# kokutoupan/burn_raymarching

Hardware: AMD Instinct MI355X
Metric: Mrays/s fwd+bwd, 512x512 / 256 spheres / 32 steps, at 1/2/4/8 MI355X (higher is better)
Workload: dtype f32

## Files before the change

burn_raymarching_amd/csrc/rm_kernels.hip:

```cpp
#include <hip/hip_runtime.h>
#include <hip/hip_ext.h>

#include <algorithm>
#include <cstdarg>
#include <cmath>
#include <cstdio>
#include <cstdlib>
#include <cstring>
#include <string>
#include <type_traits>
#include <utility>
#include <vector>

#include "../../include/raymarch.h"
#include "rm_device.h"

namespace rm {

constexpr int kOrderClasses = 16;
constexpr int kOrderClsStride = 32;
constexpr int kOrderCntStride = kOrderClasses * kOrderClsStride > 64 ? kOrderClasses * kOrderClsStride : 64;
static_assert(kOrderCntStride >= kOrderClasses * kOrderClsStride && kOrderCntStride % 32 == 0, "128-byte lines per set");
constexpr int kRedArrStride = 32;

enum Mode { kFwd = 0, kBwd = 1, kTrain = 2, kRender = 3 };

constexpr int kMaxBlocksPerLaunch = 131072 * (256 / kBlock);
constexpr int kInlineCams = 16;
constexpr int kSplitMinSpheres = 256;
constexpr int kSplitMinSpheresWide = 512;
constexpr long long kSplitMaxRaysWide = 1048576;
constexpr int kSplitMinWaves = 3;
constexpr int kSplitWaves = 4;
static_assert(kSplitWaves == 2 || kSplitWaves == 4, "split blocks have 2 or 4 waves");
constexpr int kSplitRays = 32;
static_assert(kSplitRays == 64 || kSplitRays == 32 || kSplitRays == 16, "split blocks hold 64, 32 or 16 rays");
constexpr int kSplitCB = kSplitRays / 16;
constexpr long long kSplitMaxRays = 262144;
constexpr int kReduceSegs = 128;

struct KArgs {
  const float* org;
  const float* dir;
  long long ray_begin;
  long long n_rays;
  int width, height, num_views;
  int tiling;
  int cull;
  float cull_min_d;
  float lse_slack;
  unsigned long long* stats;
  float gone_d;
  int early_exit;
  int split;
  int mfma;
  int shift_max;
  const int* esc_flags;
  const int* block_order;
  int order_views, order_tiles;
  const int* olist_r;
  const int* ocnt_r;
  int* olist_w;
  int* ocnt_w;
  int* ocnt_z;
  const int* oturn;
  CamBasis cams[kInlineCams];
  const CamBasis* cams_dev;
  const float* centers;
  const float* colors;
  const _Float16* colors_h;
  const float* radius;
  const float* light_dir;
  const float* ambient;
  int M, Mpad;
  const float4* rec_buf;
  float* origin;
  int steps;
  float k, eps, csharp, msharp;
  float* out;
  float* t_out;
  const float* t_in;
  const float* gout;
  const float* targets;
  float progress, inv_count;
  const rm_step_scalars* sdev;
  float light_fixed[3];
  float* dbg;
  float* partials;
  long long rec;
  int cont_cap, cont_resume;
  float* cont_state;
  const int* cont_list;
  const int* cont_count;
  int* cont_list_w;
  int* cont_count_w;
  long long cont_rays;
  int ray_cont;
  const int* ray_list;
  const int* ray_count;
  int* ray_list_w;
  int* ray_count_w;
#ifdef RM_BLOCK_TRACE
  unsigned long long* btrace;
#endif
};
#ifdef RM_BLOCK_TRACE
constexpr int kTraceWords = 12;
__device__ __forceinline__ void trace_word(const KArgs& a, int w, unsigned long long v) {
  if (a.btrace != nullptr && (threadIdx.x & 63) == 0)
    a.btrace[kTraceWords * ((unsigned long long)blockIdx.x * kWaves + (threadIdx.x >> 6)) + w] = v;
}
#define RM_TRACE(w, v) trace_word(a, (w), (v))
#else
#define RM_TRACE(w, v) ((void)0)
#endif

typedef float f4v __attribute__((ext_vector_type(4)));
typedef float f2v __attribute__((ext_vector_type(2)));
typedef const __attribute__((address_space(4))) f4v* cf4_ptr;
typedef const __attribute__((address_space(4))) f2v* cf2_ptr;
typedef const __attribute__((address_space(4))) float* cf1_ptr;

constexpr int kRecHeader = 8;

__host__ __device__ inline size_t tiles_offset(int npairs, int nprep) {
  return ((size_t)npairs * (7 * 16 + 8) + (size_t)(nprep + 1) * kRecHeader * sizeof(float) + 15) & ~(size_t)15;
}
constexpr int kEscTab = 64;
constexpr int kStatsWords = 6;
__host__ __device__ inline size_t esc_offset(int npairs, int nprep) {
  const size_t nrb = (size_t)npairs / 8;
  return tiles_offset(npairs, nprep) + nrb * 64 * 16 + nrb * 32 * sizeof(float);
}
__host__ __device__ inline size_t origin_offset(int npairs, int nprep) {
  return esc_offset(npairs, nprep) + kEscTab * sizeof(float);
}
// ... 81 lines not shown
      v[k] = fminf(v[k], c);
      v[3 + k] = fmaxf(v[3 + k], c);
    }
#pragma unroll
  for (int off = 32; off > 0; off >>= 1)
#pragma unroll
    for (int k = 0; k < 3; ++k) {
      v[k] = fminf(v[k], __shfl_xor(v[k], off));
      v[3 + k] = fmaxf(v[3 + k], __shfl_xor(v[3 + k], off));
    }
  if (lane == 0)
#pragma unroll
    for (int k = 0; k < 6; ++k) scratch[8 * wave + k] = v[k];
  __syncthreads();
#pragma unroll
  for (int k = 0; k < 3; ++k) {
    float lo = scratch[k], hi = scratch[3 + k];
    for (int w = 1; w < nw; ++w) {
      lo = fminf(lo, scratch[8 * w + k]);
      hi = fmaxf(hi, scratch[8 * w + 3 + k]);
    }
    c0[k] = 0.5f * (lo + hi);
  }
  float r = 0.0f;
  for (int j = tid; j < a.M; j += nt) {
    const float dx = a.centers[3 * j] - c0[0], dy = a.centers[3 * j + 1] - c0[1], dz = a.centers[3 * j + 2] - c0[2];
    r = fmaxf(r, fsqrt(dx * dx + dy * dy + dz * dz) + a.radius[j]);
  }
#pragma unroll
  for (int off = 32; off > 0; off >>= 1) r = fmaxf(r, __shfl_xor(r, off));
  __syncthreads();
  if (lane == 0) scratch[8 * wave] = r;
  __syncthreads();
  R = scratch[0];
  for (int w = 1; w < nw; ++w) R = fmaxf(R, scratch[8 * w]);
  R = R * (1.0f + 1e-5f) + 1e-6f;
  __syncthreads();
}

typedef short bf16x8 __attribute__((ext_vector_type(8)));
typedef float f32x4 __attribute__((ext_vector_type(4)));

__device__ __forceinline__ void split3(float x, unsigned& h1, unsigned& h2, unsigned& h3) {
  const unsigned a = __float_as_uint(x) & 0xFFFF0000u;
  const float r1 = x - __uint_as_float(a);
  const unsigned b = __float_as_uint(r1) & 0xFFFF0000u;
  const float r2 = r1 - __uint_as_float(b);
  const unsigned c = __float_as_uint(r2) & 0xFFFF0000u;
  h1 = a >> 16;
  h2 = b >> 16;
  h3 = c >> 16;
}
__device__ __forceinline__ unsigned pack2(unsigned lo16, unsigned hi16) { return lo16 | (hi16 << 16); }
constexpr unsigned kBf16One = 0x3F80u;

__device__ __forceinline__ uint4 mfma_a_slice(const KArgs& a, int j, int g) {
  const float kappa = a.k * kLog2e, k2 = kappa * kappa;
  float cx, cy, cz;
  if (j < a.M) {
    cx = a.centers[3 * j];
    cy = a.centers[3 * j + 1];
    cz = a.centers[3 * j + 2];
  } else {
    cx = kPadCenter;
    cy = cz = 0.0f;
  }
  unsigned x[3], y[3], z[3], C[3];
  split3(-2.0f * k2 * cx, x[0], x[1], x[2]);
  split3(-2.0f * k2 * cy, y[0], y[1], y[2]);
  split3(-2.0f * k2 * cz, z[0], z[1], z[2]);
  split3(k2 * (cx * cx + cy * cy + cz * cz), C[0], C[1], C[2]);
  if (g < 2)
    return make_uint4(pack2(x[g], x[g]), pack2(x[g], y[g]), pack2(y[g], y[g]), pack2(z[g], z[g]));
  if (g == 2) return make_uint4(pack2(x[2], x[2]), pack2(0u, y[2]), pack2(y[2], 0u), pack2(z[2], z[2]));
  return make_uint4(pack2(z[0], z[1]), pack2(kBf16One, kBf16One), pack2(kBf16One, C[0]), pack2(C[1], C[2]));
}
__device__ __forceinline__ uint4 mfma_a_frag(const KArgs& a, int e) {
  const int l = e & 63;
  return mfma_a_slice(a, 16 * (e >> 6) + (l & 15), l >> 4);
}
__device__ __forceinline__ int mfma_w_sphere(int e) { return 16 * (e >> 5) + (e & 15); }
__device__ __forceinline__ bool mfma_w_fixed(int e) { return (e & 16) != 0; }

__device__ void write_bound(const KArgs& a, float* hdr, float* esc) {
  __shared__ float scratch[8 * 16];
  float c[3], R;
  scene_bound(a, scratch, threadIdx.x, c, R);
  if (threadIdx.x == 0) {
    hdr[4] = c[0];
    hdr[5] = c[1];
    hdr[6] = c[2];
    hdr[7] = R;
  }
  if (threadIdx.x < kEscTab) {
    float tv = INFINITY;
    if (a.gone_d > 0.0f) {
      const float rp = (R + a.lse_slack + 1e-3f) * (1.0f + 1e-6f);
      const float inv_shrink = 1.0000101f;
      float T = (a.gone_d + rp) * (1.0f + 1e-6f);
      const float two_c2 = 2.0f * inv_shrink * inv_shrink * (1.0f + 1e-6f), nrp2 = -rp * rp,
                  half_up = 0.5f * (1.0f + 1e-5f);
      const int nmax = min((int)threadIdx.x, a.steps);
      for (int n = 1; n <= nmax; ++n) T = fmaf(rp + fsqrt(fmaf(two_c2 * T, T, nrp2)), half_up, 1e-6f);
      tv = T * (1.0f + 1e-6f);
    }
    esc[threadIdx.x] = tv;
  }
}

constexpr int kPrepStageMax = 512;

template <bool PAR>
__device__ void write_origins(const KArgs& a, const float4& S00, const float4& S10, float rmax, float spread,
                              const uint4* At, const float* Wt, float* orig, unsigned char* xch, int v);

__global__ __launch_bounds__(256) void rm_prep_kernel(const KArgs a0, float4* __restrict__ rec) {
  __shared__ float stage[7 * kPrepStageMax];
  const int nt = (int)blockDim.x;
  KArgs a = a0;
  if (gridDim.x == 1 && a0.M <= kPrepStageMax) {
    const int M = a0.M;
    for (int e = threadIdx.x; e < 3 * M; e += nt) {
      stage[e] = a0.centers[e];
      stage[3 * M + e] = a0.colors_h != nullptr ? (float)a0.colors_h[e] : a0.colors[e];
    }
    for (int e = threadIdx.x; e < M; e += nt) stage[6 * M + e] = a0.radius[e];
    __syncthreads();
    a.centers = stage;
    a.colors = stage + 3 * M;
    a.colors_h = nullptr;
    a.radius = stage + 6 * M;
  }
  const int np = a.Mpad / 2;
  float4* P0 = rec;
  float4* P1 = P0 + np;
  float4* P2 = P1 + np;
  float4* P3 = P2 + np;
  float4* S0 = P3 + np;
  float4* S1 = S0 + np;
  float4* W = S1 + np;
  float2* P4 = reinterpret_cast<float2*>(W + np);
  float* hdr = reinterpret_cast<float*>(P4 + np);
  const float kappa = a.k * kLog2e, k2 = kappa * kappa;
  const float kr_first = kappa * a.radius[0];
  const float c0x = a.centers[0], c0y = a.centers[1], c0z = a.centers[2];
  float rmin = INFINITY, rmax = 0.0f, spread = 0.0f;
  const int ip = blockIdx.x * nt + threadIdx.x;
  if (ip < np) {
    float gx[2], gy[2], gz[2], cc[2], kr[2], rr[2], cr[2], cg[2], cb[2], w[2], wf[2];
#pragma unroll
    for (int h = 0; h < 2; ++h) {
      const int j = 2 * ip + h;
      if (j < a.M) {
        const float cx = a.centers[3 * j], cy = a.centers[3 * j + 1], cz = a.centers[3 * j + 2];
        const float r = a.radius[j];
        gx[h] = -2.0f * cx;
        gy[h] = -2.0f * cy;
        gz[h] = -2.0f * cz;
        cc[h] = cx * cx + cy * cy + cz * cz;
        kr[h] = kappa * r;
        rr[h] = r;
        if (a.colors_h != nullptr) {
          cr[h] = (float)a.colors_h[3 * j];
          cg[h] = (float)a.colors_h[3 * j + 1];
          cb[h] = (float)a.colors_h[3 * j + 2];
        } else {
          cr[h] = a.colors[3 * j];
          cg[h] = a.colors[3 * j + 1];
          cb[h] = a.colors[3 * j + 2];
        }
        w[h] = fexp2(kr[h]);
// ... 755 lines not shown
```

burn_raymarching_amd/csrc/rm_launch.h:

```cpp
#pragma once

namespace {

using namespace rm;

int pad_spheres(int M) { return (M + kSphereAlign - 1) / kSphereAlign * kSphereAlign; }
constexpr int kRedArrivals = (RM_MAX_SPHERES * 8 + 8 + 255) / 256 * kRedArrStride;

long long max_blocks_per_launch() {
  const char* e = std::getenv("RM_MAX_BLOCKS_PER_LAUNCH");
  const long long v = e ? std::atoll(e) : 0;
  return (v >= 1 && v <= kMaxBlocksPerLaunch) ? v : kMaxBlocksPerLaunch;
}

long long rec_floats(int Mpad) { return (long long)Mpad * 8 + 8; }

int split_cont_steps(int steps) {
  if (const char* e = std::getenv("RM_SPLIT_CONT_STEPS")) return std::max(0, std::atoi(e));
  return steps >= 64 ? std::max(32, 3 * steps / 8) : 0;
}
int split_cont2_steps(int steps) {
  if (const char* e = std::getenv("RM_SPLIT_CONT2_STEPS")) return std::max(0, std::atoi(e));
  return steps >= 128 ? 3 * steps / 4 : 0;
}
// ... 433 lines not shown
}

int small_lpr(const Call& c, long long n) {
  if (c.mode != kTrain || env_is("RM_SMALL_LPR", '1')) return 1;
  return env_is("RM_SMALL_LPR", '2') || n <= 32768 ? 2 : 1;
}

int run_small(rm_context* ctx, const Call& c, KArgs& a, long long n) {
  const bool has_bwd = c.has_bwd();
  const int lpr = small_lpr(c, n), rpb = kBlock / lpr;
  int rc;
  if (has_bwd && (rc = ctx->ws.ensure(ctx, ws_need(n, a.M, rpb), "workspace")) != RM_OK) return rc;
  if ((rc = ctx->arrivals.ensure(ctx, 64, "arrival counter", true)) != RM_OK) return rc;
  long long done = 0;
  bool first = true;
  while (done < n) {
    const long long nb = std::min<long long>((n - done + rpb - 1) / rpb, max_blocks_per_launch());
    const long long nr = std::min<long long>(n - done, nb * rpb);
    a.ray_begin = done;
    a.n_rays = nr;
    a.partials = ctx->ws.as<float>();
#ifdef RM_BLOCK_TRACE
    if ((rc = bind_block_trace(ctx, a, (nb + (c.fused && c.fused->adam ? 1 : 0)) * kWaves)) != RM_OK) return rc;
    RM_HIP(ctx, hipMemsetAsync(a.btrace, 0, sizeof(unsigned long long) * kTraceWords * kWaves * (size_t)(nb + 1), ctx->stream));
#endif
    SmallArgs sa;
    std::memset(&sa, 0, sizeof sa);
    if (c.fused) sa = *c.fused;
    if (has_bwd) sa.fin = final_args(c, first);
    sa.arrivals = ctx->arrivals.as<unsigned>();
    sa.final_in_kernel = has_bwd && nb <= kSmallFinalMaxBlocks ? 1 : 0;
    if (c.fused && (!sa.final_in_kernel || nr != n))
      return fail(ctx, RM_ERR_INVALID_ARG, "fused iteration needs one launch of <= %d blocks", kSmallFinalMaxBlocks);
    const bool extra = c.fused && sa.adam;
    if (ctx->stats_dev) {
      ctx->stats_blocks += nb;
      ctx->stats_waves += nb * kWaves;
    }
    if (extra) {
      if ((rc = ctx->opt_pre.ensure(ctx, sizeof(float) * (4 * kOptPreStride + 2), "optimizer hand-off")) != RM_OK)
        return rc;
      sa.opt_pre = ctx->opt_pre.as<float>();
      ctx->opt_prepared = false;
    }
    hipEvent_t ev0, ev1;
    if ((rc = next_events(ctx, ev0, ev1)) != RM_OK) return rc;
    const dim3 grid((unsigned)(nb + (extra ? 1 : 0)));
    if (c.fused && lpr == 2) launch_small_m<kTrain, true, 2>(a.M, grid, ctx->stream, a, sa, ev0, ev1);
    else if (c.fused) launch_small_m<kTrain, true>(a.M, grid, ctx->stream, a, sa, ev0, ev1);
    else if (c.mode == kFwd) launch_small_m<kFwd>(a.M, grid, ctx->stream, a, sa, ev0, ev1);
    else if (c.mode == kBwd) launch_small_m<kBwd>(a.M, grid, ctx->stream, a, sa, ev0, ev1);
    else if (lpr == 2) launch_small_m<kTrain, false, 2>(a.M, grid, ctx->stream, a, sa, ev0, ev1);
    else launch_small_m<kTrain>(a.M, grid, ctx->stream, a, sa, ev0, ev1);
    RM_HIP(ctx, hipGetLastError());
    if (has_bwd && !sa.final_in_kernel && (rc = reduce_and_finalize(ctx, c, a, nb, first)) != RM_OK) return rc;
    done += nr;
    first = false;
  }
  return RM_OK;
}


template <int MODE>
void launch_escape(bool cam, dim3 grid, hipStream_t st, const KArgs& a, int* flags) {
  if (cam)
    hipLaunchKernelGGL((rm_escape_kernel<MODE, true>), grid, dim3(kBlock), 0, st, a, flags);
  else
    hipLaunchKernelGGL((rm_escape_kernel<MODE, false>), grid, dim3(kBlock), 0, st, a, flags);
}

template <int MODE>
bool launch_ray(bool cam, bool split, dim3 grid, size_t lds, hipStream_t st, const KArgs& a, hipEvent_t ev0,
                hipEvent_t ev1) {
  const dim3 blk(split ? 64 * kSplitWaves : kBlock);
  const uint32_t sh = (uint32_t)lds;
  if (split) {
    if constexpr (MODE == kRender) {
      return false;
    } else {
      if (cam) hipExtLaunchKernelGGL((rm_ray_kernel<MODE, true, true>), grid, blk, sh, st, ev0, ev1, 0u, a);
      else hipExtLaunchKernelGGL((rm_ray_kernel<MODE, false, true>), grid, blk, sh, st, ev0, ev1, 0u, a);
    }
  } else {
    if (cam) hipExtLaunchKernelGGL((rm_ray_kernel<MODE, true, false>), grid, blk, sh, st, ev0, ev1, 0u, a);
    else hipExtLaunchKernelGGL((rm_ray_kernel<MODE, false, false>), grid, blk, sh, st, ev0, ev1, 0u, a);
  }
  return true;
}

int check_call(rm_context* ctx, const Call& c, long long n) {
  if ((c.mode == kFwd || c.mode == kRender) && n > 0 && !c.out && !c.t_out && !c.dbg) return fail(ctx, RM_ERR_INVALID_ARG, "no output requested");
  if (c.mode == kBwd && n > 0 && !c.gout) return fail(ctx, RM_ERR_INVALID_ARG, "grad_out is NULL");
  if (c.mode == kTrain && n > 0 && !c.targets) return fail(ctx, RM_ERR_INVALID_ARG, "targets is NULL");
  if (c.has_bwd() && !c.grads) return fail(ctx, RM_ERR_INVALID_ARG, "grads is NULL");
  return RM_OK;
}

bool march_policy(const Call& c, long long n, KArgs& a) {
  const int M = a.M;
  const bool mask_vanishes = c.mode == kRender || a.msharp > 0.0f;
  bool split = false;
  if (c.mode != kRender && (c.march->flags & RM_MARCH_SKIP_ESCAPED) == 0) {
    const char* e = std::getenv("RM_SPLIT");
    if ((c.march->flags & RM_MARCH_SPLIT) != 0 || (e && e[0] == '1')) split = true;
    else if ((c.march->flags & RM_MARCH_NO_SPLIT) == 0 && !(e && e[0] == '0'))
      split = (M >= kSplitMinSpheres && n <= kSplitMaxRays) || (M >= kSplitMinSpheresWide && n <= kSplitMaxRaysWide);
  }
  a.split = split ? 1 : 0;
  a.cull = ((c.march->flags & RM_MARCH_SKIP_ESCAPED) != 0 && mask_vanishes && !c.t_out && !c.dbg && !split) ? 1 : 0;
  a.cull_min_d = c.mode == kRender ? 50.0f : std::max(50.0f, 160.0f / (a.msharp * 1.44269504f));
  a.gone_d = 0.0f;
  if (!c.dbg) {
    if (c.mode == kRender) a.gone_d = 6.0f;
    else if (a.msharp > 0.0f) a.gone_d = std::max(6.0f, 130.0f / (a.msharp * 1.44269504f));
  }
  a.early_exit = a.gone_d > 0.0f && (c.march->flags & RM_MARCH_NO_EARLY_EXIT) == 0 && !c.t_out ? 1 : 0;
  a.mfma = (c.march->flags & RM_MARCH_VALU_ONLY) == 0;
  a.shift_max = (c.march->flags & RM_MARCH_FORCE_MAX_SHIFT) != 0;
  if (c.mode == kRender) {
    const float lv[3] = {-0.5f, 0.5f, -1.0f};
    const float len = std::sqrt(lv[0] * lv[0] + lv[1] * lv[1] + lv[2] * lv[2]);
    for (int i = 0; i < 3; ++i) a.light_fixed[i] = lv[i] / len;
  }
  return split;
}

int ensure_block_order(rm_context* ctx, int tx, int ty, int sub) {
  if (ctx->block_order && ctx->order_tx == tx && ctx->order_ty == ty && ctx->order_sub == sub) return RM_OK;
  std::vector<int> ord((size_t)tx * ty * sub);
  for (size_t i = 0; i < ord.size(); ++i) ord[i] = (int)i;
  auto key = [&](int i) {
    const int tile = i / sub, q = i % sub;
    const int per_quad = sub / 4, quad = sub == 1 ? 0 : q / per_quad, part = sub == 1 ? 0 : q % per_quad;
    const long long rows = sub == 1 ? 16 : 8 / per_quad;
    const long long ox = sub == 1 ? 16 : 16 * (quad & 1) + 8,
                    oy = sub == 1 ? 16 : 16 * (quad >> 1) + 2 * rows * part + rows;
    const long long dx = 32LL * (tile % tx) + ox - 16LL * tx, dy = 32LL * (tile / tx) + oy - 16LL * ty;
    return dx * dx + dy * dy;
  };
  std::stable_sort(ord.begin(), ord.end(), [&](int x, int y) { return key(x) < key(y); });
  if (ctx->block_order) RM_HIP(ctx, hipStreamSynchronize(ctx->stream));
  int rc;
  if ((rc = ctx->block_order.ensure(ctx, sizeof(int) * ord.size(), "block order")) != RM_OK) return rc;
  RM_HIP(ctx, hipMemcpy(ctx->block_order.p, ord.data(), sizeof(int) * ord.size(), hipMemcpyHostToDevice));
  ctx->order_tx = tx;
  ctx->order_ty = ty;
  ctx->order_sub = sub;
  return RM_OK;
}

struct Launch {
  long long done, nb, nr, blocks_left;
  int rpb;
};

int bind_block_order(rm_context* ctx, const Call& c, const Launch& l, KArgs& a) {
  a.block_order = nullptr;
  const long long npix = (long long)c.W * c.H;
  if (!(c.cam && a.tiling == 2 && l.nb > 1 && l.done % npix == 0 && l.nr % npix == 0 && l.nr == l.nb * l.rpb &&
        (c.march->flags & RM_MARCH_NATURAL_ORDER) == 0))
    return RM_OK;
  int rc;
  if ((rc = ensure_block_order(ctx, c.W / 16, c.H / 16, 256 / l.rpb)) != RM_OK) return rc;
  a.block_order = ctx->block_order.as<int>();
  a.order_views = (int)(l.nr / npix);
  a.order_tiles = (int)(npix / l.rpb);
  return RM_OK;
}

int bind_cost_order(rm_context* ctx, const Call& c, const Launch& l, KArgs& a) {
  a.olist_r = nullptr;
  a.ocnt_r = nullptr;
  a.olist_w = nullptr;
  a.ocnt_w = nullptr;
  a.ocnt_z = nullptr;
  a.oturn = nullptr;
  if (!c.has_bwd()) return RM_OK;
  unsigned long long key = 0;
  if (a.block_order != nullptr && l.nb == l.blocks_left && l.done == 0 && (c.march->flags & RM_MARCH_STATIC_ORDER) == 0) {
    key = ((unsigned long long)c.W << 48) ^ ((unsigned long long)c.H << 32) ^ ((unsigned long long)c.views << 24) ^
          ((unsigned long long)a.Mpad << 1) ^ 1ull ^ ((unsigned long long)(a.split != 0) << 2);
    constexpr int kCls = kOrderClasses;
    int rc;
    if ((rc = ctx->olist.ensure(ctx, sizeof(int) * 3 * kCls * kMaxBlocksPerLaunch, "cost-order lists")) != RM_OK) return rc;
    if ((rc = ctx->ocnt.ensure(ctx, sizeof(int) * 4 * kOrderCntStride, "cost-order counts", true)) != RM_OK) return rc;
    int* olist = ctx->olist.as<int>();
    int* ocnt = ctx->ocnt.as<int>();
    ctx->oturn = ocnt + 3 * kOrderCntStride;
    if (ctx->cost_valid && ctx->cost_key == key) {
      a.olist_r = olist;
      a.ocnt_r = ocnt;
    }
    a.olist_w = olist;
    a.ocnt_w = ocnt;
    a.ocnt_z = env_is("RM_DEBUG_SKIP_ORDER_CLEAR", '1') ? nullptr : ocnt;
    a.oturn = ctx->oturn;
  }
  ctx->cost_valid = key != 0;
  ctx->cost_key = key;
// ... 301 lines not shown
```

burn_raymarching_amd/csrc/rm_ray.h:

```cpp
#pragma once

struct ContState {
  enum Row { kT = 0, kLb, kDprev, kCycT1, kCycT2, kCode, kRhoLb, kRhist, kRayRows };
  static constexpr int kGroupWords = 2;
  struct Ray {
    float t, lb, Dprev, cyc_t1, cyc_t2, rho_lb;
    int rhist;
    bool gone, retired;
  };
  float* cs;
  long long R;
  __host__ __device__ static size_t floats(long long rays, long long groups) {
    return (size_t)(kRayRows * rays + kGroupWords * groups);
  }
  __device__ __forceinline__ explicit ContState(const KArgs& a) : cs(a.cont_state), R(a.cont_rays) {}
  __device__ __forceinline__ float& row(int r, long long li) const { return cs[r * R + li]; }
  __device__ __forceinline__ float& group(long long blk, int w) const { return cs[kRayRows * R + kGroupWords * blk + w]; }
  __device__ __forceinline__ static float code(const Ray& s) { return s.gone ? 1.0f : (s.retired ? 2.0f : 0.0f); }
  __device__ __forceinline__ Ray load(long long li) const {
    Ray s;
    s.t = row(kT, li);
    s.lb = row(kLb, li);
    s.Dprev = row(kDprev, li);
    s.cyc_t1 = row(kCycT1, li);
    s.cyc_t2 = row(kCycT2, li);
    const float gflag = row(kCode, li);
    s.gone = gflag == 1.0f;
    s.retired = gflag == 2.0f;
    s.rho_lb = row(kRhoLb, li);
    s.rhist = __float_as_int(row(kRhist, li));
    return s;
  }
  __device__ __forceinline__ void save(long long li, const Ray& s) const {
    row(kT, li) = s.t;
    row(kLb, li) = s.lb;
    row(kDprev, li) = s.Dprev;
    row(kCycT1, li) = s.cyc_t1;
    row(kCycT2, li) = s.cyc_t2;
    row(kCode, li) = code(s);
    row(kRhoLb, li) = s.rho_lb;
    row(kRhist, li) = __int_as_float(s.rhist);
  }
  __device__ __forceinline__ void write_back(long long li, const Ray& s) const {
    row(kT, li) = s.t;
    row(kLb, li) = s.lb;
    row(kCode, li) = code(s);
    row(kRhoLb, li) = s.rho_lb;
  }
};

__device__ __forceinline__ Lds bind_lds(const KArgs& a, unsigned char* smem) {
  Lds L;
  const int np = a.Mpad / 2;
  L.P0 = (cf4_ptr)a.rec_buf;
  L.P1 = L.P0 + np;
  L.P2 = L.P1 + np;
  L.P3 = L.P2 + np;
  L.S0 = L.P3 + np;
  L.S1 = L.S0 + np;
  L.W = L.S1 + np;
  L.P4 = (cf2_ptr)(L.W + np);
  L.At = reinterpret_cast<const uint4*>(reinterpret_cast<const char*>(a.rec_buf) + tiles_offset(np, (np + 255) / 256));
  L.Wt = reinterpret_cast<const float*>(L.At + (size_t)(np / 8) * 64);
  L.slots = reinterpret_cast<float*>(smem);
  L.misc = L.slots + kSlotBytes / sizeof(float);
  return L;
}

struct LaneSphere {
  float gx = -2.0f * kPadCenter, gy = 0.0f, gz = 0.0f, cc = kPadCenter * kPadCenter;
  float kr = 0.0f, rr = 0.0f, cr = 0.0f, cg = 0.0f, cbl = 0.0f;
};
template <bool COLOUR>
__device__ __forceinline__ LaneSphere load_sphere(const float4* R4, const float2* R2, int np, int j, int Mpad) {
  LaneSphere s;
  if (j < Mpad) {
    const int i = j >> 1;
    const bool h = (j & 1) != 0;
    const float4 A = R4[i], B = R4[np + i], R = R4[2 * np + i];
    s.gx = h ? A.y : A.x;
    s.gy = h ? A.w : A.z;
    s.gz = h ? B.y : B.x;
    s.cc = h ? B.w : B.z;
    if constexpr (COLOUR) {
      const float4 C3 = R4[3 * np + i];
      const float2 C4 = R2[i];
      s.rr = h ? R.w : R.z;
      s.cr = h ? C3.y : C3.x;
      s.cg = h ? C3.w : C3.z;
      s.cbl = h ? C4.y : C4.x;
    } else {
      s.kr = h ? R.y : R.x;
    }
  }
  return s;
}
__device__ __forceinline__ void add_cols4(float* rec, int j, const float (&v)[8]) {
  float4* dst = reinterpret_cast<float4*>(rec + (long long)j * 8);
  float4 o = dst[0];
  o.x += v[0];
  o.y += v[1];
  o.z += v[2];
  o.w += v[3];
  dst[0] = o;
}

template <int MODE, bool CAM, bool SPLIT>
__device__ __forceinline__ void ray_body(const KArgs& a);

template <int MODE, bool CAM, bool SPLIT>
__device__ __forceinline__ void ray_entry(const KArgs& a) {
#ifdef RM_BLOCK_TRACE
  const unsigned long long t_begin = __builtin_amdgcn_s_memrealtime();
  ray_body<MODE, CAM, SPLIT>(a);
  const unsigned long long t_end = __builtin_amdgcn_s_memrealtime();
  if (a.btrace != nullptr && (threadIdx.x & 63) == 0) {
    const unsigned hw = __builtin_amdgcn_s_getreg((31 << 11) | 4);
    const unsigned xcc = __builtin_amdgcn_s_getreg((31 << 11) | 20);
    unsigned long long* r = a.btrace + kTraceWords * ((unsigned long long)blockIdx.x * kWaves + (threadIdx.x >> 6));
    r[0] = t_begin;
    r[1] = t_end;
    r[2] = (unsigned long long)hw | ((unsigned long long)xcc << 32);
    r[3] = (unsigned long long)ray_block(a) | ((unsigned long long)blockIdx.x << 32);
  }
#else
  ray_body<MODE, CAM, SPLIT>(a);
#endif
}
template <int MODE, bool CAM, bool SPLIT>
__global__ __launch_bounds__(kBlock, SPLIT ? kSplitMinWaves : kMinWavesPerSimd) void rm_ray_kernel(const KArgs a) {
  ray_entry<MODE, CAM, SPLIT>(a);
}

template <int MODE, bool CAM, bool SPLIT>
__device__ __forceinline__ void ray_body(const KArgs& a) {
  extern __shared__ __attribute__((aligned(16))) unsigned char smem[];
  const Lds L = bind_lds(a, smem);

  const int tid = threadIdx.x, lane = tid & 63, wave = __builtin_amdgcn_readfirstlane(tid >> 6);
  long long blk;
  long long li_listed = -1;
  bool listed = true;
  if (SPLIT && a.cont_resume > 0 && a.ray_cont) {
    const int n = *a.ray_count;
    const int i0 = (int)blockIdx.x * kSplitRays;
    if (i0 >= n) return;
    const int i = i0 + (lane & (kSplitRays - 1));
    listed = i < n;
    li_listed = a.ray_list[listed ? i : i0];
    blk = -1;
  } else if (SPLIT && a.cont_resume > 0) {
    if ((int)blockIdx.x >= *a.cont_count) return;
    blk = a.cont_list[blockIdx.x];
  } else {
    blk = ray_block(a);
  }
  const long long li = li_listed >= 0 ? li_listed
                                      : (SPLIT ? blk * kSplitRays + (lane & (kSplitRays - 1)) : blk * kBlock + tid);
  const bool valid = listed && li < a.n_rays;
  long long ri = a.ray_begin + (valid ? li : 0);
  const bool own_rays = !SPLIT || (wave == 0 && lane < kSplitRays);

  const float kappa = a.k * kLog2e, nkappa = -kappa, inv_kappa = 1.0f / kappa;

  float o[3], d[3];
  int view;
  setup_ray<CAM>(a, ri, o, d, view);

  if (a.ocnt_z != nullptr && blockIdx.x == 0 && tid < kOrderClasses) order_sets(a).cnt_z[tid * kOrderClsStride] = 0;
  if (a.esc_flags != nullptr && blk >= 0 && a.esc_flags[blk]) {
    if (a.stats != nullptr && tid == 0) atomicAdd(a.stats, 1ull);
    if (a.ocnt_w != nullptr && tid == 0) order_append(a, blk, 0);
    escaped_block<MODE>(a, L, blk, ri, valid, tid, lane, wave);
    return;
  }

  const cf1_ptr hdr = (cf1_ptr)(L.P4 + a.Mpad / 2);
  const float rmin = hdr[0], rmax = hdr[1], spread = hdr[2];
  const bool shift_fixed_ok = !a.shift_max && kappa * (rmax + spread) * 1.001f <= 100.0f;
  const bool shift_none_ok = !a.shift_max && kappa * rmax * 1.001f <= 30.0f;
  const float kr_first = kappa * a.radius[0];
  bool gone = false;
  bool retired = false;
  float rho_lb = -INFINITY;
  const float onorm = fabsf(o[0]) + fabsf(o[1]) + fabsf(o[2]);
  auto rho_moved = [&](float rl, float t0, float t1) {
    return rl - (fabsf(t1 - t0) * 1.000001f + 1e-6f * (1.0f + onorm + fmaxf(t0, t1)));
  };
  auto all_safe = [&](float dist_lb, float rlb) {
    return __all(dist_lb + rmin >= kSafeRho || rlb >= kSafeRho || gone) != 0;
  };
  int split_par = 0;

  auto soft_min = [&](const float p[3], bool fast, float& m, float& s) {
    m = -INFINITY;
    s = 0.0f;
    if (fast)
      lse_point<false, kShiftMax>(p, L, a.Mpad / 2, nkappa, m, s);
    else
      lse_point<true, kShiftMax>(p, L, a.Mpad / 2, nkappa, m, s);
    return -(flog2(fmaxf(s, 1e-8f)) + m) * inv_kappa;
  };
  auto split_pair = [&](int w) { return (((a.Mpad / 2) * w) / kSplitWaves) & ~7; };
  auto soft_min_split = [&](const float p[3], bool fast, float& m, float& s) {
    const int b0 = split_pair(wave), b1 = split_pair(wave + 1);
    const Lds Lq = L.from_pair(b0);
    m = -INFINITY;
    s = 0.0f;
    if (fast) lse_point<false, kShiftMax>(p, Lq, b1 - b0, nkappa, m, s);
    else lse_point<true, kShiftMax>(p, Lq, b1 - b0, nkappa, m, s);
    float* xm = L.slots;
    float* xs = L.slots + kSplitWaves * 64;
    __syncthreads();
    xm[wave * 64 + lane] = m;
    xs[wave * 64 + lane] = s;
    __syncthreads();
    float mm = xm[lane];
// ... 102 lines not shown
                  : march_d_none<true, kNcb>(p, kappa, inv_kappa, At, Wt, nq, xa, xb, xs, lane, comb, wave);
      }
#ifdef RM_BLOCK_TRACE
      tr_lse_cyc += __builtin_readcyclecounter() - tq0;
#endif
      return Dm;
    }
#ifdef RM_BLOCK_TRACE
    ++tr_vec;
#endif
    if (none || fixed) {
      const float k2 = kappa * kappa;
      const int np = a.Mpad / 2;
      float sh;
      if (none) {
        s = fast ? lse_weighted<false, false>(p, L, np, k2, sh) : lse_weighted<true, false>(p, L, np, k2, sh);
      } else {
        s = fast ? lse_weighted<false, true>(p, L, np, k2, sh) : lse_weighted<true, true>(p, L, np, k2, sh);
        m = kr_first - sh;
      }
      return -(flog2(fmaxf(s, 1e-30f)) + m) * inv_kappa;
    }
    if (fast) lse_point<false, kShiftMax>(p, L, a.Mpad / 2, nkappa, m, s);
    else lse_point<true, kShiftMax>(p, L, a.Mpad / 2, nkappa, m, s);
    return -(flog2(fmaxf(s, 1e-30f)) + m) * inv_kappa;
  };
  auto soft_min_march = [&](const float p[3], bool fast, float Dprev, int& choice, const Memo& mm) {
    if constexpr (SPLIT) {
      const bool live = !gone && !retired;
      bool nr = live && shift_none_ok && 2.0f * fmaxf(Dprev, 0.0f) + a.lse_slack <= 90.0f * inv_kappa;
      if (live && !nr && shift_none_ok && a.mfma)
        nr = fixed_shift(p, kappa * kappa, Lds::v4(L.S0[0]), Lds::v4(L.S1[0])) - kr_first <= 90.0f;
      const bool far = live && !nr && !(psq(p) <= 1e10f);
      const bool use_fixed = !nr && shift_fixed_ok && !far;
      unsigned long long bn = __ballot(nr);
      const unsigned long long bf = __ballot(live && use_fixed), bx = __ballot(live && !nr && !use_fixed);
      if (!a.early_exit && (bn | bf | bx) == 0ull) bn = 1ull;
      int cm = 0;
      float Dn = 0.0f, Dm = 0.0f, Dx = 0.0f;
      if (bn != 0ull) Dn = soft_min_core(p, fast, Dprev, cm, 3, mm);
      if (bf != 0ull) Dm = soft_min_core(p, fast, Dprev, cm, 1, mm);
      if (bx != 0ull) Dx = soft_min_core(p, fast, Dprev, cm, 2, mm);
      choice = (nr ? 1 : 0) | (use_fixed ? 2 : 0) | (fast ? 4 : 0);
      return nr ? Dn : (use_fixed ? Dm : Dx);
    } else {
      return soft_min_core(p, fast, Dprev, choice, 0, mm);
    }
  };

  float t = 0.0f;
  float lb = -INFINITY;
  float Dprev = INFINITY;
  bool dead = false;
  int steps_saved = 0;
  const float c0x = hdr[4], c0y = hdr[5], c0z = hdr[6];
  const cf1_ptr esc_tab = (cf1_ptr)(reinterpret_cast<const char*>(a.rec_buf) + esc_offset(a.Mpad / 2, (a.Mpad / 2 + 255) / 256));
  if (MODE == kBwd && a.t_in != nullptr) {
    t = a.t_in[ri];
  } else {
    const float rprime = (hdr[7] + a.lse_slack + 1e-3f) * (1.0f + 1e-6f);
    float gone_step = 0.0f;
    auto wave_escaped = [&](int st, const float p[3]) {
      if (!(a.gone_d > 0.0f)) return false;
      const float ex = p[0] - c0x, ey = p[1] - c0y, ez = p[2] - c0z;
      const float Tn = esc_tab[min(a.steps - st, kEscTab - 1)];
      const float dist = fsqrt(fmaf(ez, ez, fmaf(ey, ey, ex * ex)));
      gone = gone || (!retired && fmaf(ez, d[2], fmaf(ey, d[1], ex * d[0])) >= 0.0f && dist * (1.0f - 1e-5f) >= Tn);
      gone_step = dist - rprime;
      if (a.early_exit && __all(gone || !valid)) {
        steps_saved += a.steps - st;
        return true;
      }
      return false;
    };
    auto gone_steps = [&](int from) {
      for (int k = from; k < a.steps; ++k) {
        const float q[3] = {fmaf(d[0], t, o[0]) - c0x, fmaf(d[1], t, o[1]) - c0y, fmaf(d[2], t, o[2]) - c0z};
        t = fminf(t + (fsqrt(fmaf(q[2], q[2], fmaf(q[1], q[1], q[0] * q[0]))) - rprime), kTMax);
      }
    };
    auto gone_finish = [&](int from) {
      if (gone && !retired) gone_steps(from);
    };
    int st_stop = -1;
    int st0 = 0;
#ifdef RM_BLOCK_TRACE
    const unsigned long long tr_c_begin = __builtin_readcyclecounter();
    unsigned long long tr_cyc = 0;
#endif
    if constexpr (CAM) {
      if (a.origin != nullptr && a.steps > 0 && !(SPLIT && a.cont_resume > 0)) {
        const float D0 = a.origin[view];
        rho_lb = a.origin[RM_MAX_VIEWS_PER_CALL + view];
        if (__all((__float_as_uint(D0) & 0x7fffffffu) <= 0x7f800000u)) {
          const float p[3] = {fmaf(d[0], t, o[0]), fmaf(d[1], t, o[1]), fmaf(d[2], t, o[2])};
          if (wave_escaped(0, p)) {
            dead = true;
          } else {
            t = fminf(t + (gone ? gone_step : D0), kTMax);
            rho_lb = rho_moved(rho_lb, 0.0f, t);
            lb = D0 - fabsf(D0);
            Dprev = D0;
            st0 = 1;
            steps_saved = 1;
          }
        }
      }
    }
    float cyc_t1 = __builtin_nanf(""), cyc_t2 = __builtin_nanf("");
    int chist = 0xFFF;
    float Dprev2 = INFINITY;
    int rhist = 0xFFF;
    if (SPLIT && a.cont_resume > 0) {
      const ContState cs(a);
      const ContState::Ray s = cs.load(li);
      t = s.t;
      lb = s.lb;
      Dprev = s.Dprev;
      cyc_t1 = s.cyc_t1;
      cyc_t2 = s.cyc_t2;
      gone = s.gone;
      retired = s.retired;
      rho_lb = s.rho_lb;
      rhist = s.rhist;
      if (!a.ray_cont) {
        chist = __float_as_int(cs.group(blk, 0));
        steps_saved = __float_as_int(cs.group(blk, 1));
      }
      st0 = a.cont_resume;
    }
    const unsigned long long below = (1ull << lane) - 1ull;
    for (int st = st0; !dead && st < a.steps; ++st) {
      if (SPLIT && a.cont_cap > 0 && st == a.cont_cap) {
        const ContState cs(a);
        const bool act = valid && !gone && !retired && lane < kSplitRays;
        gone_finish(st);
        if (wave == 0 && lane < kSplitRays && valid)
          cs.save(li, ContState::Ray{t, lb, Dprev, cyc_t1, cyc_t2, rho_lb, rhist, gone, retired});
        if (wave == 0) {
          const unsigned long long am = __ballot(act);
          const int na = __popcll(am);
          int base = 0;
          if (lane == 0 && na > 0) base = atomicAdd(a.ray_count_w, na);
          base = __shfl(base, 0);
          if (act) a.ray_list_w[base + __popcll(am & below)] = (int)li;
          if (lane == 0) {
            if (!a.ray_cont) {
              cs.group(blk, 0) = __int_as_float(chist);
              cs.group(blk, 1) = __int_as_float(steps_saved + (a.steps - st));
              a.cont_list_w[atomicAdd(a.cont_count_w, 1)] = (int)blk;
            } else if (a.stats != nullptr && st > st0) {
              atomicAdd(a.stats + 2, (unsigned long long)(-(long long)(st - st0)));
            }
          }
        }
        return;
      }
      const float p[3] = {fmaf(d[0], t, o[0]), fmaf(d[1], t, o[1]), fmaf(d[2], t, o[2])};
      if (wave_escaped(st, p)) {
        dead = true;
        st_stop = st;
        break;
      }
      int choice;
      const Memo mm{t, cyc_t1, cyc_t2, Dprev2, chist};
      const float D = soft_min_march(p, all_safe(lb, rho_lb), Dprev, choice, mm);
      const float t_step = t;
      if constexpr (SPLIT) {
        const float rl0 = rho_lb;
        if (!retired) {
          t = fminf(t + (gone ? gone_step : D), kTMax);
          rho_lb = rho_moved(rl0, t_step, t);
          lb = D - fabsf(D);
          Dprev = D;
        }
        if (a.early_exit && MODE != kRender) {
          if (!retired && !gone && valid && t_step == cyc_t2 && (choice & 3) == ((rhist >> 3) & 3)) {
            retired = true;
            if (((a.steps - st) & 1) == 0) {
              t = t_step;
              rho_lb = rl0;
            }
          }
          if (!retired) {
            cyc_t2 = cyc_t1;
            cyc_t1 = t_step;
          }
          rhist = ((rhist << 3) | choice) & 0xFFF;
          if (__all(gone || !valid || retired)) {
            if (gone) gone_steps(st + 1);
            steps_saved += a.steps - 1 - st;
            break;
          }
        }
        continue;
      }
      t = fminf(t + (gone ? gone_step : D), kTMax);
      rho_lb = rho_moved(rho_lb, t_step, t);
      lb = D - fabsf(D);
      Dprev2 = Dprev;
      Dprev = D;
      if (a.early_exit && MODE != kRender) {
        if (choice == ((chist >> 3) & 7) && __all(gone || t_step == cyc_t2)) {
          constexpr int P = 2;
          const int left = a.steps - 1 - st, m = a.steps - st, back = (P - m % P) % P;
          const int cf = back == 0 ? choice : (chist >> (3 * (back - 1))) & 7;
          if (!gone) {
            if (back == 0) t = t_step;
            else if (back == 1) t = cyc_t1;
            lb = (cf & 4) ? INFINITY : -INFINITY;
            rho_lb = -INFINITY;
          } else {
// ... 547 lines not shown
```

Baseline: 2000.

## Add soft-radius escape proof to skip marching for provably escaping waves

Adds a per-call soft (log-sum-exp) bounding radius computed in write_bound and a new PROOF kernel variant for unsplit training calls with at least 128 spheres. Before marching, each wave runs a cheap conservative sphere-trace against that bound to prove every ray escapes within the remaining steps, and if so marks the wave dead and skips the full march. This aims to remove the per-step sphere evaluation for waves that never hit geometry. In exchange it adds a pre-pass per wave, an extra reduction over spheres, and another kernel instantiation, and correctness depends on the bound being conservative.

```diff
diff --git a/burn_raymarching_amd/csrc/rm_kernels.hip b/burn_raymarching_amd/csrc/rm_kernels.hip
--- a/burn_raymarching_amd/csrc/rm_kernels.hip
+++ b/burn_raymarching_amd/csrc/rm_kernels.hip
@@ -52,6 +52,7 @@
   unsigned long long* stats;
   float gone_d;
   int early_exit;
+  int proof;
   int split;
   int mfma;
   int shift_max;
@@ -299,11 +300,35 @@
 __device__ __forceinline__ int mfma_w_sphere(int e) { return 16 * (e >> 5) + (e & 15); }
 __device__ __forceinline__ bool mfma_w_fixed(int e) { return (e & 16) != 0; }
 
+constexpr int kProofMinSpheres = 128;
+__device__ __forceinline__ float soft_radius(const KArgs& a, float* scratch, int tid, const float c0[3], float R) {
+  const int lane = tid & 63, wave = tid >> 6, nt = (int)blockDim.x, nw = nt >> 6;
+  const float kappa = a.k * kLog2e;
+  float s = 0.0f;
+  for (int j = tid; j < a.M; j += nt) {
+    const float dx = a.centers[3 * j] - c0[0], dy = a.centers[3 * j + 1] - c0[1], dz = a.centers[3 * j + 2] - c0[2];
+    const float v = (fsqrt(dx * dx + dy * dy + dz * dz) + a.radius[j]) * (1.0f + 1e-5f) + 1e-6f;
+    s += fexp2(kappa * fminf(v - R, 0.0f));
+  }
+#pragma unroll
+  for (int off = 32; off > 0; off >>= 1) s += __shfl_xor(s, off);
+  if (lane == 0) scratch[8 * wave] = s;
+  __syncthreads();
+  float sum = scratch[0];
+  for (int w = 1; w < nw; ++w) sum += scratch[8 * w];
+  __syncthreads();
+  const float rs = (R + flog2(fmaxf(sum, 1.0f) * (1.0f + 1e-5f)) / kappa) * (1.0f + 1e-5f) + 1e-6f;
+  return fminf(rs, R + a.lse_slack);
+}
+
 __device__ void write_bound(const KArgs& a, float* hdr, float* esc) {
   __shared__ float scratch[8 * 16];
   float c[3], R;
   scene_bound(a, scratch, threadIdx.x, c, R);
+  const float rsoft = a.proof ? soft_radius(a, scratch, threadIdx.x, c, R)
+                                                                    : R + a.lse_slack;
   if (threadIdx.x == 0) {
+    hdr[3] = rsoft;
     hdr[4] = c[0];
     hdr[5] = c[1];
     hdr[6] = c[2];
diff --git a/burn_raymarching_amd/csrc/rm_launch.h b/burn_raymarching_amd/csrc/rm_launch.h
--- a/burn_raymarching_amd/csrc/rm_launch.h
+++ b/burn_raymarching_amd/csrc/rm_launch.h
@@ -539,6 +539,13 @@
       else hipExtLaunchKernelGGL((rm_ray_kernel<MODE, false, true>), grid, blk, sh, st, ev0, ev1, 0u, a);
     }
   } else {
+    if constexpr (MODE != kRender) {
+      if (a.proof) {
+        if (cam) hipExtLaunchKernelGGL((rm_ray_kernel<MODE, true, false, true>), grid, blk, sh, st, ev0, ev1, 0u, a);
+        else hipExtLaunchKernelGGL((rm_ray_kernel<MODE, false, false, true>), grid, blk, sh, st, ev0, ev1, 0u, a);
+        return true;
+      }
+    }
     if (cam) hipExtLaunchKernelGGL((rm_ray_kernel<MODE, true, false>), grid, blk, sh, st, ev0, ev1, 0u, a);
     else hipExtLaunchKernelGGL((rm_ray_kernel<MODE, false, false>), grid, blk, sh, st, ev0, ev1, 0u, a);
   }
@@ -572,6 +579,7 @@
     else if (a.msharp > 0.0f) a.gone_d = std::max(6.0f, 130.0f / (a.msharp * 1.44269504f));
   }
   a.early_exit = a.gone_d > 0.0f && (c.march->flags & RM_MARCH_NO_EARLY_EXIT) == 0 && !c.t_out ? 1 : 0;
+  a.proof = a.early_exit && !split && c.mode != kRender && a.Mpad >= kProofMinSpheres ? 1 : 0;
   a.mfma = (c.march->flags & RM_MARCH_VALU_ONLY) == 0;
   a.shift_max = (c.march->flags & RM_MARCH_FORCE_MAX_SHIFT) != 0;
   if (c.mode == kRender) {
diff --git a/burn_raymarching_amd/csrc/rm_ray.h b/burn_raymarching_amd/csrc/rm_ray.h
--- a/burn_raymarching_amd/csrc/rm_ray.h
+++ b/burn_raymarching_amd/csrc/rm_ray.h
@@ -105,14 +105,14 @@
   dst[0] = o;
 }
 
-template <int MODE, bool CAM, bool SPLIT>
+template <int MODE, bool CAM, bool SPLIT, bool PROOF>
 __device__ __forceinline__ void ray_body(const KArgs& a);
 
-template <int MODE, bool CAM, bool SPLIT>
+template <int MODE, bool CAM, bool SPLIT, bool PROOF>
 __device__ __forceinline__ void ray_entry(const KArgs& a) {
 #ifdef RM_BLOCK_TRACE
   const unsigned long long t_begin = __builtin_amdgcn_s_memrealtime();
-  ray_body<MODE, CAM, SPLIT>(a);
+  ray_body<MODE, CAM, SPLIT, PROOF>(a);
   const unsigned long long t_end = __builtin_amdgcn_s_memrealtime();
   if (a.btrace != nullptr && (threadIdx.x & 63) == 0) {
     const unsigned hw = __builtin_amdgcn_s_getreg((31 << 11) | 4);
@@ -124,15 +124,16 @@
     r[3] = (unsigned long long)ray_block(a) | ((unsigned long long)blockIdx.x << 32);
   }
 #else
-  ray_body<MODE, CAM, SPLIT>(a);
+  ray_body<MODE, CAM, SPLIT, PROOF>(a);
 #endif
 }
-template <int MODE, bool CAM, bool SPLIT>
+template <int MODE, bool CAM, bool SPLIT, bool PROOF = false>
 __global__ __launch_bounds__(kBlock, SPLIT ? kSplitMinWaves : kMinWavesPerSimd) void rm_ray_kernel(const KArgs a) {
-  ray_entry<MODE, CAM, SPLIT>(a);
+  static_assert(!PROOF || (!SPLIT && MODE != kRender), "the escape proof: unsplit training kernels");
+  ray_entry<MODE, CAM, SPLIT, PROOF>(a);
 }
 
-template <int MODE, bool CAM, bool SPLIT>
+template <int MODE, bool CAM, bool SPLIT, bool PROOF>
 __device__ __forceinline__ void ray_body(const KArgs& a) {
   extern __shared__ __attribute__((aligned(16))) unsigned char smem[];
   const Lds L = bind_lds(a, smem);
@@ -401,6 +402,27 @@
     auto gone_finish = [&](int from) {
       if (gone && !retired) gone_steps(from);
     };
+    constexpr float kProofMinStep = 0.02f;
+    auto bound_proof = [&](int st) {
+      if (__any(!(onorm + fabsf(c0x) + fabsf(c0y) + fabsf(c0z) + 3.0f * esc_tab[0] <= 256.0f))) return false;
+      const float rs = (hdr[3] + 1e-3f) * (1.0f + 1e-6f) + 1e-3f;
+      float u = t;
+      bool proven = gone || !valid;
+      for (int n = st; n < a.steps; ++n) {
+        const float ex = fmaf(d[0], u, o[0]) - c0x, ey = fmaf(d[1], u, o[1]) - c0y, ez = fmaf(d[2], u, o[2]) - c0z;
+        const float dist = fsqrt(fmaf(ez, ez, fmaf(ey, ey, ex * ex)));
+        const float Tn = esc_tab[min(a.steps - n, kEscTab - 1)];
+        proven = proven || (fmaf(ez, d[2], fmaf(ey, d[1], ex * d[0])) >= 0.0f && dist * (1.0f - 2e-5f) >= Tn);
+        if (__all(proven)) {
+          steps_saved += a.steps - st;
+          return true;
+        }
+        const float Lb = dist - rs;
+        if (__any(!proven && !(Lb > kProofMinStep))) return false;
+        u += proven ? 0.0f : Lb;
+      }
+      return false;
+    };
     int st_stop = -1;
     int st0 = 0;
 #ifdef RM_BLOCK_TRACE
@@ -447,6 +469,9 @@
         steps_saved = __float_as_int(cs.group(blk, 1));
       }
       st0 = a.cont_resume;
+    }
+    if constexpr (PROOF) {
+      if (!dead && bound_proof(st0)) dead = true;
     }
     const unsigned long long below = (1ull << lane) - 1ull;
     for (int st = st0; !dead && st < a.steps; ++st) {
```

New measurement: 2080, median of 6. 1.04x the previous value.
